# bjack205/altro

Measured on AMD Instinct MI355X. Metric: iLQR backward+forward sweeps/sec (N knotpoints x batch), higher is better.
Workload: dtype f64

## Files before the change

altro_amd/__init__.py:

```python
import ctypes as C
import os

import numpy as np

_HERE = os.path.dirname(os.path.abspath(__file__))
LIB_PATH = os.path.join(_HERE, "lib", "libaltro_hip.so")

F64, F32 = 0, 1
PLAN_AUTO, PLAN_GENERIC, PLAN_MFMA16, PLAN_LANE, PLAN_MFMA32 = 0, 1, 2, 3, 4
STORE_QBLOCKS = 0x1
LANE_FUSED = 0x4
F32_PURE = 0x2
TILE_USER_BLOCKS = 0x2
GENERIC_MATRIX_CORES = 0x8
TVLQR_SUCCESS = -1

C_ABI_SYMBOLS = [
    "altro_hip_version", "altro_hip_last_error", "altro_hip_device_count", "altro_hip_device_info", "altro_hip_device_pci_bus_id",
    "altro_hip_batch_create", "altro_hip_batch_create_dims", "altro_hip_batch_destroy", "altro_hip_batch_plan",
    "altro_hip_batch_device_bytes", "altro_hip_set_dynamics", "altro_hip_set_cost",
    "altro_hip_set_initial_state", "altro_hip_set_host_batch", "altro_hip_backward", "altro_hip_forward_ltv", "altro_hip_sweep",
    "altro_hip_synchronize", "altro_hip_get_K", "altro_hip_get_d", "altro_hip_get_P",
    "altro_hip_get_p", "altro_hip_get_x", "altro_hip_get_u", "altro_hip_get_y",
    "altro_hip_get_delta_V", "altro_hip_get_status", "altro_hip_get_qblocks",
    "altro_hip_stats_reduce", "altro_hip_comm_unique_id", "altro_hip_comm_create", "altro_hip_comm_create_all",
    "altro_hip_comm_destroy", "altro_hip_comm_rank", "altro_hip_comm_world", "altro_hip_comm_device", "altro_hip_stats_allreduce", "altro_hip_stats_allreduce_multi",
    "altro_hip_profile_enable", "altro_hip_profile_reset",
    "altro_hip_profile_get", "altro_hip_profile_get_range", "altro_hip_profile_dropped", "altro_hip_algorithmic_bytes",
    "altro_hip_set_model", "altro_hip_set_model_source", "altro_hip_model_row_layout", "altro_hip_set_tracking_cost", "altro_hip_set_quadratic_cost",
    "altro_hip_set_input_guess", "altro_hip_set_state_guess",
    "altro_hip_open_loop_rollout", "altro_hip_accept", "altro_hip_expand", "altro_hip_merit", "altro_hip_merit_affine",
    "altro_hip_stationarity", "altro_hip_get_nominal", "altro_hip_get_expansion",
    "altro_hip_default_solve_options", "altro_hip_set_forms", "altro_hip_get_forms", "altro_hip_ilqr_solve", "altro_hip_last_solve_counts",
    "altro_hip_ilqr_solve_async", "altro_hip_ilqr_poll", "altro_hip_ilqr_wait",
    "altro_hip_linesearch_host",
    "altro_hip_add_linear_constraint", "altro_hip_add_user_constraint", "altro_hip_clear_constraints", "altro_hip_reset_duals",
    "altro_hip_get_duals", "altro_hip_set_duals", "altro_hip_get_penalty", "altro_hip_set_penalty", "altro_hip_shift_duals", "altro_hip_feasibility",
    "altro_hip_shift_trajectory", "altro_hip_update_linear_costs", "altro_hip_get_knot",
    "altro_hip_set_pointer_mode",
]
CONE_EQUALITY, CONE_IDENTITY, CONE_INEQUALITY, CONE_SOC = 0, 1, 2, 3

DUAL_TAIL_KEEP, DUAL_TAIL_ZERO = 0, 1
FORM_NO_SPECULATION, FORM_NO_RUNAHEAD, FORM_NO_MERIT2, FORM_MERIT_LDS, FORM_MERIT_DPP_ALWAYS = 0x1, 0x2, 0x4, 0x8, 0x10
FORM_EXPAND_LDS, FORM_ALROWS_LDS, FORM_ROLLOUT_ROUNDS, FORM_SEQUENCED, FORM_MERIT_ONE_LAUNCH = 0x20, 0x40, 0x80, 0x100, 0x200
FORM_LANE_QUAD_OFF, FORM_LANE_QUAD_ON, FORM_GENERIC_LATE_Q_OFF, FORM_GENERIC_LATE_Q_ON, FORM_FUSED_CLOCK = 0x400, 0x800, 0x1000, 0x2000, 0x4000
FORM_AFFINE_EXACT = 0x8000
FORM_NO_COMPACTION = 0x10000
FORM_GENERIC_MERIT_LDS = 0x20000


def forms_from_env():
    e = os.environ
    off = lambda name: e.get(name) is not None and e[name].strip() not in ("",) and _atoi(e[name]) == 0
    f = 0
    if "ALTRO_HIP_NO_SPECULATION" in e: f |= FORM_NO_SPECULATION
    if "ALTRO_HIP_NO_RUNAHEAD" in e and not off("ALTRO_HIP_NO_RUNAHEAD"): f |= FORM_NO_RUNAHEAD
    if off("ALTRO_HIP_MERIT2"): f |= FORM_NO_MERIT2
    if off("ALTRO_HIP_MERIT_DPP"): f |= FORM_MERIT_LDS
    elif e.get("ALTRO_HIP_MERIT_DPP") is not None and _atoi(e["ALTRO_HIP_MERIT_DPP"]) == 2: f |= FORM_MERIT_DPP_ALWAYS
    if off("ALTRO_HIP_EXPAND_DPP"): f |= FORM_EXPAND_LDS
    if off("ALTRO_HIP_ALROWS_DPP"): f |= FORM_ALROWS_LDS
    if off("ALTRO_HIP_AFFINE"): f |= FORM_ROLLOUT_ROUNDS
    if off("ALTRO_HIP_FUSED") or "ALTRO_HIP_NO_FUSED" in e: f |= FORM_SEQUENCED
    if off("ALTRO_HIP_MERIT_SPLIT"): f |= FORM_MERIT_ONE_LAUNCH
    if "ALTRO_HIP_LANE_QUAD" in e: f |= FORM_LANE_QUAD_OFF if _atoi(e["ALTRO_HIP_LANE_QUAD"]) == 0 else FORM_LANE_QUAD_ON
    if "ALTRO_HIP_GENERIC_LATE_Q" in e: f |= FORM_GENERIC_LATE_Q_OFF if _atoi(e["ALTRO_HIP_GENERIC_LATE_Q"]) == 0 else FORM_GENERIC_LATE_Q_ON
    if "ALTRO_HIP_FUSED_CLOCK" in e: f |= FORM_FUSED_CLOCK
    if "ALTRO_HIP_AFFINE_EXACT" in e: f |= FORM_AFFINE_EXACT
    if "ALTRO_HIP_NO_COMPACTION" in e: f |= FORM_NO_COMPACTION
    return f


def _atoi(text):
    try:
        return int(text.strip() or 0)
    except ValueError:
        return 0

MODEL_LINEAR, MODEL_DOUBLE_INTEGRATOR, MODEL_PENDULUM, MODEL_BICYCLE, MODEL_USER, MODEL_QUADROTOR, MODEL_QUADROTOR13 = 0, 1, 2, 3, 4, 5, 6
MERIT_FN = C.CFUNCTYPE(None, C.c_double, C.POINTER(C.c_double), C.POINTER(C.c_double), C.c_void_p)

# ... 576 lines not shown
```

altro_amd/csrc/capi_core.hip:

```cpp
#include "capi_internal.h"

namespace altro_hip {
namespace capi {

thread_local std::string g_last_error;

int fail(int code, const char* fmt, ...) {
  char buf[512];
  va_list ap;
  va_start(ap, fmt);
  vsnprintf(buf, sizeof(buf), fmt, ap);
  va_end(ap);
  g_last_error = buf;
  return code;
}

}
}

using namespace altro_hip;
using namespace altro_hip::capi;

namespace {

// ... 581 lines not shown
  if (h->prof_n == 0) return 0;
  int rc = check(h);
  if (rc) return rc;
  HIP_TRY(hipStreamSynchronize(h->stream));
  for (int i = 0; i < h->prof_n; ++i) {
    float ms = 0.f;
    if (hipEventElapsedTime(&ms, h->prof_ev[2 * i], h->prof_ev[2 * i + 1]) != hipSuccess) continue;
    const int slot = h->prof_slot[i];
    h->prof_min[slot] = h->prof_launches[slot] ? std::min(h->prof_min[slot], (double)ms) : (double)ms;
    h->prof_max[slot] = std::max(h->prof_max[slot], (double)ms);
    h->prof_ms[slot] += ms;
    h->prof_launches[slot] += 1;
  }
  h->prof_n = 0;
  return 0;
}
}
int altro_hip_profile_get(altro_hip_batch* h, int slot, int* launches, double* total_ms,
                          const char** kernel_name) {
  if (!h || slot < 0 || slot > 1) return fail(ALTRO_HIP_ERR_BAD_ARGUMENT, "bad handle or slot");
  int rc = profile_drain(h);
  if (rc) return rc;
  if (launches) *launches = h->prof_launches[slot];
  if (total_ms) *total_ms = h->prof_ms[slot];
  if (kernel_name) {
    static const char* names[3][2] = {{"generic_backward_kernel", "generic_forward_kernel"},
                                      {"mfma16_backward_kernel", "mfma16_forward_kernel"},
                                      {"lane_backward_kernel", "lane_forward_kernel"}};
    *kernel_name = names[h->plan == ALTRO_HIP_PLAN_MFMA16 ? 1 : (h->plan == ALTRO_HIP_PLAN_LANE ? 2 : 0)][slot];
    if (h->g_tile && !(slot == 0 && h->is_diag)) *kernel_name = slot == 0 ? "tile32_backward_kernel" : "tile32_forward_kernel";
    if (slot == 0 && h->plan == ALTRO_HIP_PLAN_LANE && h->bwd_quad) *kernel_name = h->n == 4 ? "quad_backward_kernel" : "quad2_backward_kernel";
    if (slot == 1 && h->plan == ALTRO_HIP_PLAN_LANE && h->fwd_quad) *kernel_name = "quad_forward_kernel";
    if (slot == 1 && mfma16_forward_is_x4(h)) *kernel_name = "mfma16_forward_f32x4_kernel";
    if (slot == 0 && h->plan == ALTRO_HIP_PLAN_MFMA16 && h->dtype == ALTRO_HIP_F32 && (h->flags & ALTRO_HIP_F32_PURE) &&
        !(h->flags & ALTRO_HIP_STORE_QBLOCKS))
      *kernel_name = (h->batch % 4 == 0) ? "mfma16_backward_f32x4_kernel"
                                                                                    : "mfma16_backward_f32_kernel";
  }
  return 0;
}
int altro_hip_profile_dropped(altro_hip_batch* h, int slot) {
  if (!h || slot < 0 || slot > 1) return fail(ALTRO_HIP_ERR_BAD_ARGUMENT, "bad handle or slot");
  return h->prof_dropped[slot];
}
int altro_hip_profile_get_range(altro_hip_batch* h, int slot, double* min_ms, double* max_ms) {
  if (!h || slot < 0 || slot > 1) return fail(ALTRO_HIP_ERR_BAD_ARGUMENT, "bad handle or slot");
  int rc = profile_drain(h);
  if (rc) return rc;
  if (min_ms) *min_ms = h->prof_min[slot];
  if (max_ms) *max_ms = h->prof_max[slot];
  return 0;
}

double altro_hip_algorithmic_bytes(const altro_hip_batch* h, int slot) {
  if (!h) return 0.0;
  const double n = h->n, m = h->m, w = (double)h->esz;
  const double bwd = 3 * n * n + 3 * n * m + m * m + 3 * n + 2 * m;
  const double fwd = 2 * n * n + 2 * n * m + 4 * n + 2 * m;
  return (slot == 0 ? bwd : fwd) * w * (double)h->N * (double)h->batch;
}

}
```

altro_amd/csrc/capi_internal.h:

```cpp
#pragma once
#include "altro_hip/altro_hip.h"

#include <hip/hip_runtime.h>
#include <hip/hip_ext.h>

#include <algorithm>
#include <cstdarg>
#include <cstdio>
#include <cstdlib>
#include <cstring>
#include <string>
#include <vector>

#include "kernels/pack.hip"
#include "kernels/tvlqr_generic.hip"
#include "kernels/tvlqr_lane.hip"
#include "kernels/ilqr_types.h"
#include "kernels/ilqr_generic.hip"
#include "kernels/mfma16_layout.h"
#include "linesearch_sm.h"
#include "al_tables.h"
#include "al_shift.h"
#include "loop_fields.h"
#include "loop_route.h"
// ... 19 lines not shown

using namespace altro_hip;

struct altro_hip_batch {
  int N = 0, n = 0, m = 0, batch = 0, dtype = 0, plan = 0, device = 0;
  unsigned flags = 0;
  unsigned forms = 0;
  hipStream_t stream = nullptr;
  bool own_stream = false;
  size_t esz = 8;
  void* x0 = nullptr;
  void* delta_V = nullptr;
  int* status = nullptr;
  bool dyn_set = false, cost_set = false, x0_set = false, backward_done = false, forward_done = false;
  int has_f = 0, is_diag = 0;
  int host_batch = 0;
  bool dev_ptrs = false;
  void* g_arr[G_NUM] = {};
  int64_t g_bstride[G_NUM] = {};
  void *i_sens = nullptr, *i_sens_alpha = nullptr, *i_aff_part = nullptr, *i_aff_on = nullptr;
  bool aff_failed = false;
  bool aff_enabled = false, aff_round = false, aff_store = false;
  bool aff_base = false;
  bool g_tile = false;
  bool g_mfma = false;
  bool ragged = false;
  std::vector<int> nxv, nuv;
  int64_t* g_off = nullptr;
  int* g_nx = nullptr;
  int* g_nu = nullptr;
  void *m_in = nullptr, *m_cin = nullptr, *m_term = nullptr, *m_out = nullptr, *m_outn = nullptr, *m_xuy = nullptr,
       *m_qblk = nullptr, *m_trash = nullptr;
  Mfma16Strides m_st{};
  void *l_in = nullptr, *l_term = nullptr, *l_out = nullptr, *l_outn = nullptr, *l_xuy = nullptr,
       *l_x0 = nullptr;
  void *l_nom = nullptr, *l_cost = nullptr;
  IlqrProb* i_prob = nullptr;
  double *i_alpha = nullptr, *i_phi = nullptr, *i_dphi = nullptr;
  int *i_active = nullptr, *i_counters = nullptr;
  int* cnt_host = nullptr;
  int* cnt_host_dev = nullptr;
  hipEvent_t cnt_ev[16] = {};
  void* i_cand_spec = nullptr;
  void* poll_host = nullptr; int* poll_count_host = nullptr;
  bool async_request = false, async_pending = false;
  bool rtc_row32_ok = false;
  bool rtc_has_constraints = false;
  void* rtc = nullptr;
  std::string rtc_source;
  int rtc_ck = 0;
  int x0_stride = 0;
  int spare_count = 0;
  int spare_failed = 0;
  int *i_spec_sel = nullptr, *i_spec_refresh = nullptr;
  int* i_fused_list = nullptr;
  int fused_resident = 0;
  int *i_guard = nullptr, *i_active_exact = nullptr;
  int* i_stat_done = nullptr;
  const int* stat_skip = nullptr;
  void *i_merit_jk = nullptr, *i_spec_jac = nullptr;
  int merit_split = -1;
  void *i_results = nullptr, *i_results_host = nullptr;
  void* g_ws = nullptr;
  bool fwd_quad = false;
  bool bwd_quad = false;
  int spec_trials = 1;
// ... 385 lines not shown
inline int field_get(altro_hip_batch* h, const LoopShape& s, int field, int k0, int nk, double* host) {
  const FieldRef r = field_run(s, field, k0, &nk);
  if (r.kind == LK_LANE) return lane_get(h, host, loop_buffer(h, r.buf), k0 * r.ks, nullptr, r.E, (int)r.off, 0, r.len, nk, nk);
  return aos_get(h, host, loop_buffer(h, r.buf), r.off, r.bs, r.ks, r.len, nk);
}

constexpr int kCounterSlots = 2048;
constexpr int kStatsBlocks = 1024, kStatsStride = 16;

int rtc_current(altro_hip_batch* h, const RouteShape& s);
int rtc_step(altro_hip_batch* h, const RouteStep& st, const void* args);
RouteShape route_shape(const altro_hip_batch* h);

int replan_empty_handle(altro_hip_batch* h, int plan);
int al_upload(altro_hip_batch* h);
int model_takes_dynamics(altro_hip_batch* h);
int ilqr_check(altro_hip_batch* h, bool need_guess);
int ilqr_run(altro_hip_batch* h, int which, bool use_alpha, bool use_active, int want_deriv, double alpha_const,
             int mode = EXPAND_GRADIENT | EXPAND_HESSIAN);
template <typename T>
IlqrArgs<T> ilqr_args(altro_hip_batch* h, bool use_alpha, bool use_active, int want_deriv, double alpha_const);
int spec_trials_cap(const altro_hip_batch* h);
bool merit_rounds_dpp(const altro_hip_batch* h);
bool affine_eligible(const altro_hip_batch* h);
bool affine_buffers(altro_hip_batch* h);
bool ensure_spares(altro_hip_batch* h, int count, size_t bytes_each);
void merit_split_prepare(altro_hip_batch* h);
int ilqr_gather_results(altro_hip_batch* h, altro_hip_solve_result* results);
int launch_backward(altro_hip_batch* h, double reg);
bool tile32_supported(int n, int m);
int tile32_launch_backward(altro_hip_batch* h, double reg);
int tile32_launch_forward(altro_hip_batch* h);
int launch_forward(altro_hip_batch* h);
bool mfma16_forward_is_x4(const altro_hip_batch* h);

}
int al_shift_duals_launch(hipStream_t stream, void* z, int esz, const int* order, const int* start, int nchains, int batch, int tail);
int al_set_penalty_launch(hipStream_t stream, IlqrProb* prob, const double* rho, int stride, int batch);
int al_get_penalty_launch(hipStream_t stream, const IlqrProb* prob, double* rho, int batch);
namespace capi {

}
}
```

altro_amd/csrc/capi_tvlqr.hip:

```cpp
#include "capi_internal.h"
#include "models.h"

#include "kernels/tvlqr_mfma16.hip"
#include "kernels/tvlqr_mfma16_f32.hip"
#include "kernels/tvlqr_mfma16_f32x4.hip"
#include "kernels/tvlqr_mfma16_fwd_f32x4.hip"

using namespace altro_hip;
using namespace altro_hip::capi;

#define PROF_LAUNCH(kernel, grid, block, lds, stream, ...) \
  hipExtLaunchKernelGGL(kernel, grid, block, lds, stream, h->launch_ev0, h->launch_ev1, 0, __VA_ARGS__)

namespace {

template <typename T>
int lane_launch(altro_hip_batch* h, bool backward, double reg) {
  LaneArgs<T> a{(const T*)h->l_in, (const T*)h->l_term, (T*)h->l_out, (T*)h->l_outn, (const T*)h->l_x0,
                (T*)h->l_xuy, (T*)h->delta_V, h->status, h->N, h->batch, (T)reg, backward ? h->bwd_active : nullptr,
                backward ? h->bwd_reg : nullptr};
  const dim3 grid(8 * (((h->batch + 63) / 64 + 7) / 8)), block(64);
  const bool fused = (h->flags & ALTRO_HIP_LANE_FUSED) != 0;
  const bool quad_on = form(h, ALTRO_HIP_FORM_LANE_QUAD_ON) ? true : form(h, ALTRO_HIP_FORM_LANE_QUAD_OFF) ? false : h->batch <= 12288;
  const bool q42 = h->n == 4 && h->m == 2, q21 = h->n == 2 && h->m == 1;
  if (backward) h->bwd_quad = quad_on && (q42 || q21);
  if (!backward) h->fwd_quad = quad_on && q42;
  if (!backward && quad_on && q42) {
    const dim3 qgrid(8 * (((h->batch + 15) / 16 + 7) / 8));
    if (fused) PROF_LAUNCH((quad_forward_kernel_fused<2, T>), qgrid, block, 0, h->stream, a);
    else PROF_LAUNCH((quad_forward_kernel<2, T>), qgrid, block, 0, h->stream, a);
    hipError_t e = hipGetLastError();
    if (e != hipSuccess) return fail(ALTRO_HIP_ERR_HIP, "quad kernel launch: %s", hipGetErrorString(e));
    return 0;
  }
  if (backward && h->bwd_quad) {
    const dim3 qgrid(8 * (((h->batch + 15) / 16 + 7) / 8));
    if (q42 && fused) PROF_LAUNCH((quad_backward_kernel_fused<2, T>), qgrid, block, 0, h->stream, a);
    else if (q42) PROF_LAUNCH((quad_backward_kernel<2, T>), qgrid, block, 0, h->stream, a);
    else if (fused) PROF_LAUNCH((quad2_backward_kernel_fused<T>), qgrid, block, 0, h->stream, a);
// ... 73 lines not shown
    }
    h->launch_ev0 = nullptr; h->launch_ev1 = nullptr;
  }
};


template <typename S>
Mfma16Args<S> mfma16_args(altro_hip_batch* h, double reg) {
  Mfma16Args<S> a;
  a.in = (const S*)h->m_in;
  a.cin = (const S*)h->m_cin;
  a.cin_bs = h->m_st.cin_bs; a.cin_ks = h->m_st.cin_ks;
  a.in_bs = h->m_st.in_bs; a.in_ks = h->m_st.in_ks; a.out_bs = h->m_st.out_bs; a.out_ks = h->m_st.out_ks;
  a.xuy_bs = h->m_st.xuy_bs; a.xuy_ks = h->m_st.xuy_ks;
  a.term = (const S*)h->m_term; a.out = (S*)h->m_out; a.outn = (S*)h->m_outn; a.qblk = (S*)h->m_qblk;
  a.trash = (S*)h->m_trash; a.x0 = (const S*)h->x0; a.xuy = (S*)h->m_xuy; a.delta_V = (S*)h->delta_V;
  a.status = h->status; a.N = h->N; a.batch = h->batch; a.reg = reg; a.has_f = h->has_f && !h->ilqr_linear;
  a.active = h->bwd_active; a.reg_pp = h->bwd_reg;
  return a;
}
template <typename S>
void mfma16_launch_backward(altro_hip_batch* h, double reg, bool sq) {
  auto a = mfma16_args<S>(h, reg);
  const dim3 grid(mf_grid(h->batch)), block(64);
  if (sq && a.has_f) PROF_LAUNCH((mfma16_backward_kernel<true, true, S>), grid, block, 0, h->stream, a);
  else if (sq) PROF_LAUNCH((mfma16_backward_kernel<true, false, S>), grid, block, 0, h->stream, a);
  else if (a.has_f) PROF_LAUNCH((mfma16_backward_kernel<false, true, S>), grid, block, 0, h->stream, a);
  else PROF_LAUNCH((mfma16_backward_kernel<false, false, S>), grid, block, 0, h->stream, a);
}

template <typename S>
void mfma16_launch_forward(altro_hip_batch* h, const Mfma16Args<S>& a) {
  PROF_LAUNCH((mfma16_forward_kernel<S, 3>), dim3(mf_grid(h->batch)), dim3(64), 0, h->stream, a);
}

}

namespace altro_hip {
namespace capi {

int launch_backward(altro_hip_batch* h, double reg) {
  ProfScope ps(h, 0);
  h->aff_base = false;
  if (h->plan == ALTRO_HIP_PLAN_MFMA16) {
    const bool sq = (h->flags & ALTRO_HIP_STORE_QBLOCKS) != 0;
    if (h->dtype == ALTRO_HIP_F64) mfma16_launch_backward<double>(h, reg, sq);
    else if (sq || !(h->flags & ALTRO_HIP_F32_PURE)) mfma16_launch_backward<float>(h, reg, sq);
    else {
      auto a = mfma16_args<float>(h, reg);
      if (h->batch % 4 == 0) {
        const dim3 grid(mf_grid(h->batch / 4));
        if (a.has_f) PROF_LAUNCH((mfma16_backward_f32x4_kernel<true, 2, 2>), grid, dim3(64), 0, h->stream, a);
        else PROF_LAUNCH((mfma16_backward_f32x4_kernel<false, 2, 2>), grid, dim3(64), 0, h->stream, a);
      } else if (a.has_f) PROF_LAUNCH((mfma16_backward_f32_kernel<true, 3>), dim3(mf_grid(h->batch)), dim3(64), 0, h->stream, a);
      else PROF_LAUNCH((mfma16_backward_f32_kernel<false, 3>), dim3(mf_grid(h->batch)), dim3(64), 0, h->stream, a);
    }
  } else if (h->plan == ALTRO_HIP_PLAN_LANE) {
    return h->dtype == ALTRO_HIP_F64 ? lane_launch<double>(h, true, reg) : lane_launch<float>(h, true, reg);
  } else if (h->g_tile && !h->is_diag) {
    int rc = tile32_launch_backward(h, reg);
    if (rc) return rc;
  } else {
    const bool f64 = h->dtype == ALTRO_HIP_F64;
    const size_t lds4 = f64 ? generic_backward_lds_bytes<double>(h->n, h->m) : generic_backward_lds_bytes<float>(h->n, h->m);
    const size_t lds3 = f64 ? generic_backward_lds_bytes<double>(h->n, h->m, true) : generic_backward_lds_bytes<float>(h->n, h->m, true);
    const auto per_cu = [](size_t lds) { return (int)std::min<size_t>(16, (160 * 1024) / std::max<size_t>(lds, 1)); };
// ... 6 lines not shown
    const bool big = lds > kGenericLdsLimit;
    if (big && !h->g_ws) {
      int rc = dmalloc(h, &h->g_ws, (size_t)h->batch * ((lds + 15) / 16 * 16));
      if (rc) return rc;
    }
    if (f64) {
      auto a = generic_args<double>(h, reg);
      a.ws = (double*)h->g_ws; a.ws_stride = (int64_t)((lds + 15) / 16 * 16 / sizeof(double));
      const dim3 grid(h->batch), blk(64);
      if (h->g_mfma) {
        if (big) PROF_LAUNCH((generic_backward_kernel<double, true, true>), grid, blk, 0, h->stream, a);
        else if (late_q) PROF_LAUNCH((generic_backward_kernel<double, false, true, true>), grid, blk, lds, h->stream, a);
        else PROF_LAUNCH((generic_backward_kernel<double, false, true>), grid, blk, lds, h->stream, a);
      } else if (big) PROF_LAUNCH((generic_backward_kernel<double, true>), grid, blk, 0, h->stream, a);
      else if (late_q) PROF_LAUNCH((generic_backward_kernel<double, false, false, true>), grid, blk, lds, h->stream, a);
      else PROF_LAUNCH((generic_backward_kernel<double, false>), grid, blk, lds, h->stream, a);
    } else {
      auto a = generic_args<float>(h, reg);
      a.ws = (float*)h->g_ws; a.ws_stride = (int64_t)((lds + 15) / 16 * 16 / sizeof(float));
      if (big) PROF_LAUNCH((generic_backward_kernel<float, true>), dim3(h->batch), dim3(64), 0, h->stream, a);
      else if (late_q) PROF_LAUNCH((generic_backward_kernel<float, false, false, true>), dim3(h->batch), dim3(64), lds, h->stream, a);
      else PROF_LAUNCH((generic_backward_kernel<float, false>), dim3(h->batch), dim3(64), lds, h->stream, a);
    }
  }
  hipError_t e = hipGetLastError();
  if (e != hipSuccess) return fail(ALTRO_HIP_ERR_HIP, "backward launch: %s", hipGetErrorString(e));
  return 0;
}

bool mfma16_forward_is_x4(const altro_hip_batch* h) {
  return h->plan == ALTRO_HIP_PLAN_MFMA16 && h->dtype == ALTRO_HIP_F32 && (h->flags & ALTRO_HIP_F32_PURE) && h->batch % 4 == 0;
}

int launch_forward(altro_hip_batch* h) {
  ProfScope ps(h, 1);
  h->expansion_current = false;
  if (h->plan == ALTRO_HIP_PLAN_MFMA16) {
    if (h->dtype == ALTRO_HIP_F64) {
      auto a = mfma16_args<double>(h, 0.0);
      mfma16_launch_forward<double>(h, a);
    } else {
      auto a = mfma16_args<float>(h, 0.0);
      if (mfma16_forward_is_x4(h)) {
        const dim3 grid(mf_grid(h->batch / 4));
        PROF_LAUNCH((mfma16_forward_f32x4_kernel<2, 2>), grid, dim3(64), 0, h->stream, a);
      } else {
        mfma16_launch_forward<float>(h, a);
      }
    }
  } else if (h->plan == ALTRO_HIP_PLAN_LANE) {
    return h->dtype == ALTRO_HIP_F64 ? lane_launch<double>(h, false, 0.0) : lane_launch<float>(h, false, 0.0);
  } else if (h->g_tile) {
    int rc = tile32_launch_forward(h);
    if (rc) return rc;
  } else if (h->dtype == ALTRO_HIP_F64) {
    auto a = generic_args<double>(h, 0.0);
    const size_t staged = generic_forward_lds_bytes(h->n, h->m, a.want_y, sizeof(double));
    if (staged <= kGenericForwardStageLimit) PROF_LAUNCH((generic_forward_kernel<double, true>), dim3(h->batch), dim3(64), staged, h->stream, a);
    else PROF_LAUNCH((generic_forward_kernel<double, false>), dim3(h->batch), dim3(64), (size_t)(2 * h->n + h->m) * sizeof(double) + 64, h->stream, a);
  } else {
    auto a = generic_args<float>(h, 0.0);
    const size_t staged = generic_forward_lds_bytes(h->n, h->m, a.want_y, sizeof(float));
    if (staged <= kGenericForwardStageLimit) PROF_LAUNCH((generic_forward_kernel<float, true>), dim3(h->batch), dim3(64), staged, h->stream, a);
    else PROF_LAUNCH((generic_forward_kernel<float, false>), dim3(h->batch), dim3(64), (size_t)(2 * h->n + h->m) * sizeof(float) + 64, h->stream, a);
  }
  hipError_t e = hipGetLastError();
  if (e != hipSuccess) return fail(ALTRO_HIP_ERR_HIP, "forward launch: %s", hipGetErrorString(e));
  return 0;
}

}
}

// ... 110 lines not shown
```

altro_amd/csrc/kernels/tvlqr_mfma16.hip:

```cpp
#pragma once
#include <hip/hip_runtime.h>
#include <stdint.h>

#include "mfma16_layout.h"

namespace altro_hip {

typedef double f64x4 __attribute__((ext_vector_type(4)));

__device__ __forceinline__ f64x4 mfma_f64_16x16x4(double a, double b, f64x4 c) {
  return __builtin_amdgcn_mfma_f64_16x16x4f64(a, b, c, 0, 0, 0);
}

template <int CTRL>
__device__ __forceinline__ double dpp_mov_f64(double v) {
  union { double d; int i[2]; } in, out;
  in.d = v;
  out.i[0] = __builtin_amdgcn_update_dpp(in.i[0], in.i[0], CTRL, 0xf, 0xf, false);
  out.i[1] = __builtin_amdgcn_update_dpp(in.i[1], in.i[1], CTRL, 0xf, 0xf, false);
  return out.d;
}
__device__ __forceinline__ double row16_allreduce(double v) {
  v += dpp_mov_f64<0xB1>(v);
  v += dpp_mov_f64<0x4E>(v);
// ... 275 lines not shown
}
typedef float mf_f32x4 __attribute__((ext_vector_type(4)));
struct Mfma16FwdRegsF32 {
  mf_f32x4 dyn, out;
};
__device__ __forceinline__ void mfma16_fwd_load(Mfma16FwdRegsF32& r, const float* __restrict__ rec, const float* __restrict__ orec,
                                                int lane) {
  static_assert(MF_DYN % 4 == 0 && MF_OUT % 4 == 0 && MF_OFF_F % 4 == 0, "16-byte chunks never straddle a block");
  const int cd = lane < MF_DYN / 4 ? lane : MF_DYN / 4 - 1, co = lane < MF_OUT / 4 ? lane : MF_OUT / 4 - 1;
  r.dyn = *reinterpret_cast<const mf_f32x4*>(rec + 4 * cd);
  r.out = *reinterpret_cast<const mf_f32x4*>(orec + 4 * co);
}
__device__ __forceinline__ void mfma16_fwd_stage(const Mfma16FwdRegsF32& r, double* __restrict__ L, int lane) {
  const int cd = lane < MF_DYN / 4 ? lane : MF_DYN / 4 - 1, co = lane < MF_OUT / 4 ? lane : MF_OUT / 4 - 1;
  const int e = 4 * cd;
  const int base = e < MF_OFF_F ? (e >> 4) * MF_FWD_ZLD + (e & 15) : MF_FWD_F0 + (e - MF_OFF_F);
#pragma unroll
  for (int q = 0; q < 4; ++q) L[base + q] = (double)r.dyn[q];
#pragma unroll
  for (int q = 0; q < 4; ++q) L[MF_FWD_OUT0 + 4 * co + q] = (double)r.out[q];
}
template <typename S>
struct Mfma16FwdRing { using type = Mfma16FwdRegs; };
template <>
struct Mfma16FwdRing<float> { using type = Mfma16FwdRegsF32; };
__device__ __forceinline__ double readlane_f64(double v, int src_lane) {
  union { double d; int i[2]; } in, out;
  in.d = v;
  out.i[0] = __builtin_amdgcn_readlane(in.i[0], src_lane);
  out.i[1] = __builtin_amdgcn_readlane(in.i[1], src_lane);
  return out.d;
}

template <typename S, int DEPTH>
__global__ __launch_bounds__(64) void mfma16_forward_kernel(Mfma16Args<S> a) {
  __shared__ __attribute__((aligned(16))) double lds[MF_FWD_LDS + 4];
  __shared__ double xu_lds[16];
  const int lane = threadIdx.x;
  const int b = mf_problem(blockIdx.x, a.batch);
  if (b >= a.batch) return;
  const int N = a.N;
  const S* __restrict__ in = a.in + (size_t)b * a.in_bs;
  const S* __restrict__ out = a.out + (size_t)b * a.out_bs;
  S* __restrict__ xuy = a.xuy + (size_t)b * a.xuy_bs;
  S* __restrict__ trash = a.trash + (size_t)b * MF_OUT;
  const int grp = lane >> 4;
  const int sub = lane & 15;
  const int row = (grp == 1) ? (sub < 4 ? sub : 3) : (sub < 12 ? sub : 11);
  const int row_base = (grp == 0) ? MF_FWD_ZLD * row : MF_FWD_OUT0 + 13 * (grp == 1 ? row : 0);
  int ra[13];
#pragma unroll
  for (int jj = 0; jj < 12; ++jj) ra[jj] = (grp >= 2) ? MF_FWD_OUT0 + MF_OFF_P + mf_sym(row, jj) : row_base + jj;
  ra[12] = (grp >= 2) ? MF_FWD_OUT0 + MF_OFF_p + row : row_base + 12;
  const int out_off = (grp == 0) ? row : ((grp == 1) ? 24 + row : 12 + row);
  const bool is_x = (grp == 0), is_u = (grp == 1);

  double xcur = (double)a.x0[(size_t)b * 12 + row];
  typename Mfma16FwdRing<S>::type ring[DEPTH];
#pragma unroll
  for (int dd = 0; dd < DEPTH; ++dd) {
    const int kk = (dd < N) ? dd : N - 1;
    mfma16_fwd_load(ring[dd], in + (size_t)kk * a.in_ks, out + (size_t)kk * a.out_ks, lane);
  }
  __builtin_amdgcn_s_waitcnt(0x0F70);
  mfma16_fwd_stage(ring[0], lds, lane);
  __syncthreads();

  const int Npad = ((N + DEPTH - 1) / DEPTH) * DEPTH;
  for (int k0 = 0; k0 < Npad; k0 += DEPTH) {
#pragma unroll
    for (int dd = 0; dd < DEPTH; ++dd) {
      const int k = k0 + dd;
      const bool live = k < N;
      {
        const int kn = (k + DEPTH < N) ? k + DEPTH : N - 1;
        mfma16_fwd_load(ring[dd], in + (size_t)kn * a.in_ks, out + (size_t)kn * a.out_ks, lane);
      }
      double rd[16];
#pragma unroll
      for (int j = 0; j < 13; ++j) rd[j] = lds[ra[j]];
#pragma unroll
      for (int j = 13; j < 16; ++j) rd[j] = lds[row_base + j];
      const double fi = lds[MF_FWD_F0 + row];
      double xs[12];
      if constexpr (sizeof(S) == 4) {
        if (lane < 12) xu_lds[lane] = xcur;
        __builtin_amdgcn_s_waitcnt(0xC07F);
#pragma unroll
        for (int j = 0; j < 12; ++j) xs[j] = xu_lds[j];
      } else {
#pragma unroll
        for (int j = 0; j < 12; ++j) xs[j] = readlane_f64(xcur, j);
      }
      double acc = 0.0;
#pragma unroll
      for (int j = 0; j < 12; ++j) acc = __builtin_fma(rd[j], xs[j], acc);
      const double aff = acc + rd[12];
      const double uval = -aff;
      double us[4];
      if constexpr (sizeof(S) == 4) {
        if (lane >= 16 && lane < 20) xu_lds[lane - 4] = uval;
        __builtin_amdgcn_s_waitcnt(0xC07F);
#pragma unroll
        for (int c = 0; c < 4; ++c) us[c] = xu_lds[12 + c];
      } else {
#pragma unroll
        for (int c = 0; c < 4; ++c) us[c] = readlane_f64(uval, 16 + c);
      }
      double xn = acc + fi;
#pragma unroll
      for (int c = 0; c < 4; ++c) xn = __builtin_fma(rd[12 + c], us[c], xn);
      const double sval = is_x ? xcur : (is_u ? uval : aff);
      __syncthreads();
      mfma16_fwd_stage(ring[(dd + 1) % DEPTH], lds, lane);
      S* __restrict__ o = live ? xuy + (size_t)k * a.xuy_ks : trash;
      o[out_off] = (S)sval;
      __syncthreads();
      xcur = live ? xn : xcur;
    }
  }
  {
    const S* __restrict__ on = a.outn + (size_t)b * MF_TERM;
    double xs[12];
#pragma unroll
    for (int j = 0; j < 12; ++j) xs[j] = readlane_f64(xcur, j);
    double acc = (double)on[row * 13 + 12];
#pragma unroll
    for (int j = 0; j < 12; ++j) acc = __builtin_fma((double)on[row * 13 + j], xs[j], acc);
    const double sval = is_x ? xcur : (is_u ? 0.0 : acc);
    xuy[(size_t)N * a.xuy_ks + out_off] = (S)sval;
  }
}

__global__ void mfma16_selftest_kernel(const double* A, const double* B, const double* C, double* D) {
  const int lane = threadIdx.x, j = lane & 15, g = lane >> 4;
  f64x4 c;
#pragma unroll
  for (int r = 0; r < 4; ++r) c[r] = C[(g + 4 * r) * 16 + j];
  f64x4 d = mfma_f64_16x16x4(A[j * 4 + g], B[g * 16 + j], c);
#pragma unroll
  for (int r = 0; r < 4; ++r) D[(g + 4 * r) * 16 + j] = d[r];
}

}
```

include/altro_hip/altro_hip.h:

```cpp
#ifndef ALTRO_HIP_H_
#define ALTRO_HIP_H_

#include <stddef.h>
#include <stdint.h>

#ifdef __cplusplus
extern "C" {
#endif

#define ALTRO_HIP_VERSION 300
#define ALTRO_HIP_TVLQR_SUCCESS (-1)

typedef struct altro_hip_batch altro_hip_batch;

typedef enum altro_hip_dtype {
  ALTRO_HIP_F64 = 0,
  ALTRO_HIP_F32 = 1
} altro_hip_dtype;

typedef enum altro_hip_error {
  ALTRO_HIP_OK = 0,
  ALTRO_HIP_ERR_NO_DEVICE = -1,
  ALTRO_HIP_ERR_BAD_ARGUMENT = -2,
  ALTRO_HIP_ERR_UNSUPPORTED = -3,
// ... 110 lines not shown
  double tol_stationarity;
  double tol_primal_feasibility;
  double tol_meritfun_gradient;
  int use_backtracking_linesearch;
  double penalty_initial;
  double penalty_scaling;
  double penalty_max;
  double reg_initial;
  int reg_retry_max;
  double reg_scale, reg_min, reg_max;
  int stop_when_running_at_most;
  unsigned forms;
  int fused_sweeps;
  double decision_margin;
} altro_hip_solve_options;
#define ALTRO_HIP_FORM_NO_SPECULATION 0x0001u
#define ALTRO_HIP_FORM_NO_RUNAHEAD 0x0002u
#define ALTRO_HIP_FORM_NO_MERIT2 0x0004u
#define ALTRO_HIP_FORM_MERIT_LDS 0x0008u
#define ALTRO_HIP_FORM_MERIT_DPP_ALWAYS 0x0010u
#define ALTRO_HIP_FORM_EXPAND_LDS 0x0020u
#define ALTRO_HIP_FORM_ALROWS_LDS 0x0040u
#define ALTRO_HIP_FORM_ROLLOUT_ROUNDS 0x0080u
#define ALTRO_HIP_FORM_SEQUENCED 0x0100u
#define ALTRO_HIP_FORM_MERIT_ONE_LAUNCH 0x0200u
#define ALTRO_HIP_FORM_LANE_QUAD_OFF 0x0400u
#define ALTRO_HIP_FORM_LANE_QUAD_ON 0x0800u
#define ALTRO_HIP_FORM_GENERIC_LATE_Q_OFF 0x1000u
#define ALTRO_HIP_FORM_GENERIC_LATE_Q_ON 0x2000u
#define ALTRO_HIP_FORM_AFFINE_EXACT 0x8000u
#define ALTRO_HIP_FORM_FUSED_CLOCK 0x4000u
#define ALTRO_HIP_FORM_NO_COMPACTION 0x10000u
#define ALTRO_HIP_FORM_GENERIC_MERIT_LDS 0x20000u
int altro_hip_set_forms(altro_hip_batch* h, unsigned forms);
unsigned altro_hip_get_forms(const altro_hip_batch* h);
typedef struct altro_hip_solve_result {
  int status;
  int iterations;
  double stationarity;
  double final_alpha;
  double final_phi;
  double primal_feasibility;
  double penalty;
  int dual_updates;
  int reg_retries;
} altro_hip_solve_result;
void altro_hip_default_solve_options(altro_hip_solve_options* opts);
int altro_hip_ilqr_solve(altro_hip_batch* h, const altro_hip_solve_options* opts,
                         altro_hip_solve_result* results);
int altro_hip_last_solve_counts(const altro_hip_batch* h, int* sweeps, int* merit_launches);

typedef struct altro_hip_poll_record {
  altro_hip_solve_result result;
  double u0[4];
  int done;
  int reserved;
} altro_hip_poll_record;
int altro_hip_ilqr_solve_async(altro_hip_batch* h, const altro_hip_solve_options* opts);
int altro_hip_ilqr_poll(altro_hip_batch* h, int* n_done, const altro_hip_poll_record** records);
int altro_hip_ilqr_wait(altro_hip_batch* h, altro_hip_solve_result* results);

typedef void (*altro_hip_merit_fn)(double alpha, double* phi, double* dphi, void* ctx);
double altro_hip_linesearch_host(altro_hip_merit_fn f, void* ctx, double alpha0, double phi0, double dphi0,
                                 int try_cubic_first, int use_backtracking, double c1, double c2,
                                 int* status, int* iters, double* phi, double* dphi);

// ... 41 lines not shown
```

Before: 2.710 million.

## Add grouped fp64 MFMA16 forward kernel with cooperative coalesced record loads

Adds a forward-rollout kernel where 16 waves, each handling one batch problem, cooperatively load the contiguous dynamics and output records for all 16 problems as 16-byte chunks. The records go through a two-slot LDS ring with one block barrier per step, then each wave copies its own record into a private LDS image. This replaces per-wave strided loads with wide coalesced loads across adjacent batch entries. In exchange it adds block-wide barriers, larger dynamic LDS use and lower occupancy per block. It is selected by default for f64 MFMA16 when batch is a multiple of 16 and strides are packed; a new form flag restores the single-wave path, and the shared step code is factored into helpers.

Result: faster. 2.779 million (median of 6 runs) (+2.5%).

```diff
diff --git a/altro_amd/__init__.py b/altro_amd/__init__.py
--- a/altro_amd/__init__.py
+++ b/altro_amd/__init__.py
@@ -48,6 +48,7 @@
 FORM_AFFINE_EXACT = 0x8000
 FORM_NO_COMPACTION = 0x10000
 FORM_GENERIC_MERIT_LDS = 0x20000
+FORM_FORWARD_WAVE = 0x40000
 
 
 def forms_from_env():
diff --git a/altro_amd/csrc/capi_core.hip b/altro_amd/csrc/capi_core.hip
--- a/altro_amd/csrc/capi_core.hip
+++ b/altro_amd/csrc/capi_core.hip
@@ -637,6 +637,7 @@
     if (slot == 0 && h->plan == ALTRO_HIP_PLAN_LANE && h->bwd_quad) *kernel_name = h->n == 4 ? "quad_backward_kernel" : "quad2_backward_kernel";
     if (slot == 1 && h->plan == ALTRO_HIP_PLAN_LANE && h->fwd_quad) *kernel_name = "quad_forward_kernel";
     if (slot == 1 && mfma16_forward_is_x4(h)) *kernel_name = "mfma16_forward_f32x4_kernel";
+    if (slot == 1 && mfma16_forward_is_group(h)) *kernel_name = "mfma16_forward_group_kernel";
     if (slot == 0 && h->plan == ALTRO_HIP_PLAN_MFMA16 && h->dtype == ALTRO_HIP_F32 && (h->flags & ALTRO_HIP_F32_PURE) &&
         !(h->flags & ALTRO_HIP_STORE_QBLOCKS))
       *kernel_name = (h->batch % 4 == 0) ? "mfma16_backward_f32x4_kernel"
diff --git a/altro_amd/csrc/capi_internal.h b/altro_amd/csrc/capi_internal.h
--- a/altro_amd/csrc/capi_internal.h
+++ b/altro_amd/csrc/capi_internal.h
@@ -75,6 +75,7 @@
   void *m_in = nullptr, *m_cin = nullptr, *m_term = nullptr, *m_out = nullptr, *m_outn = nullptr, *m_xuy = nullptr,
        *m_qblk = nullptr, *m_trash = nullptr;
   Mfma16Strides m_st{};
+  bool fwd_group_ready = false;
   void *l_in = nullptr, *l_term = nullptr, *l_out = nullptr, *l_outn = nullptr, *l_xuy = nullptr,
        *l_x0 = nullptr;
   void *l_nom = nullptr, *l_cost = nullptr;
@@ -526,6 +527,7 @@
 int tile32_launch_backward(altro_hip_batch* h, double reg);
 int tile32_launch_forward(altro_hip_batch* h);
 int launch_forward(altro_hip_batch* h);
+bool mfma16_forward_is_group(const altro_hip_batch* h);
 bool mfma16_forward_is_x4(const altro_hip_batch* h);
 
 }
diff --git a/altro_amd/csrc/capi_tvlqr.hip b/altro_amd/csrc/capi_tvlqr.hip
--- a/altro_amd/csrc/capi_tvlqr.hip
+++ b/altro_amd/csrc/capi_tvlqr.hip
@@ -5,6 +5,7 @@
 #include "kernels/tvlqr_mfma16_f32.hip"
 #include "kernels/tvlqr_mfma16_f32x4.hip"
 #include "kernels/tvlqr_mfma16_fwd_f32x4.hip"
+#include "kernels/tvlqr_mfma16_fwd_group.hip"
 
 using namespace altro_hip;
 using namespace altro_hip::capi;
@@ -144,6 +145,19 @@
 template <typename S>
 void mfma16_launch_forward(altro_hip_batch* h, const Mfma16Args<S>& a) {
   PROF_LAUNCH((mfma16_forward_kernel<S, 3>), dim3(mf_grid(h->batch)), dim3(64), 0, h->stream, a);
+}
+
+constexpr int kFwdGroup = 16, kFwdGroupDepth = 2;
+int mfma16_launch_forward_group(altro_hip_batch* h, const Mfma16Args<double>& a) {
+  const auto kernel = mfma16_forward_group_kernel<double, kFwdGroup, kFwdGroupDepth>;
+  const size_t lds = Mfma16FwdGroup<kFwdGroup>::lds_bytes(kFwdGroupDepth);
+  if (!h->fwd_group_ready) {
+    hipError_t e = hipFuncSetAttribute((const void*)kernel, hipFuncAttributeMaxDynamicSharedMemorySize, (int)lds);
+    if (e != hipSuccess) return fail(ALTRO_HIP_ERR_HIP, "forward group kernel: %s", hipGetErrorString(e));
+    h->fwd_group_ready = true;
+  }
+  PROF_LAUNCH(kernel, dim3(mf_grid(h->batch / kFwdGroup)), dim3(64 * kFwdGroup), lds, h->stream, a);
+  return 0;
 }
 
 }
@@ -216,13 +230,25 @@
   return h->plan == ALTRO_HIP_PLAN_MFMA16 && h->dtype == ALTRO_HIP_F32 && (h->flags & ALTRO_HIP_F32_PURE) && h->batch % 4 == 0;
 }
 
+bool mfma16_forward_is_group(const altro_hip_batch* h) {
+  const int64_t B = h->batch;
+  return h->plan == ALTRO_HIP_PLAN_MFMA16 && h->dtype == ALTRO_HIP_F64 && !form(h, ALTRO_HIP_FORM_FORWARD_WAVE) &&
+         h->batch % kFwdGroup == 0 && h->m_st.in_bs == MF_DYN && h->m_st.in_ks == B * MF_DYN && h->m_st.out_bs == MF_OUT &&
+         h->m_st.out_ks == B * MF_OUT;
+}
+
 int launch_forward(altro_hip_batch* h) {
   ProfScope ps(h, 1);
   h->expansion_current = false;
   if (h->plan == ALTRO_HIP_PLAN_MFMA16) {
     if (h->dtype == ALTRO_HIP_F64) {
       auto a = mfma16_args<double>(h, 0.0);
-      mfma16_launch_forward<double>(h, a);
+      if (mfma16_forward_is_group(h)) {
+        int rc = mfma16_launch_forward_group(h, a);
+        if (rc) return rc;
+      } else {
+        mfma16_launch_forward<double>(h, a);
+      }
     } else {
       auto a = mfma16_args<float>(h, 0.0);
       if (mfma16_forward_is_x4(h)) {
diff --git a/altro_amd/csrc/kernels/tvlqr_mfma16.hip b/altro_amd/csrc/kernels/tvlqr_mfma16.hip
--- a/altro_amd/csrc/kernels/tvlqr_mfma16.hip
+++ b/altro_amd/csrc/kernels/tvlqr_mfma16.hip
@@ -331,6 +331,78 @@
   return out.d;
 }
 
+struct Mfma16FwdRole {
+  int row, row_base, out_off;
+  int ra[13];
+  bool is_x, is_u;
+};
+__device__ __forceinline__ Mfma16FwdRole mfma16_fwd_role(int lane) {
+  Mfma16FwdRole ro;
+  const int grp = lane >> 4;
+  const int sub = lane & 15;
+  ro.row = (grp == 1) ? (sub < 4 ? sub : 3) : (sub < 12 ? sub : 11);
+  ro.row_base = (grp == 0) ? MF_FWD_ZLD * ro.row : MF_FWD_OUT0 + 13 * (grp == 1 ? ro.row : 0);
+#pragma unroll
+  for (int jj = 0; jj < 12; ++jj) ro.ra[jj] = (grp >= 2) ? MF_FWD_OUT0 + MF_OFF_P + mf_sym(ro.row, jj) : ro.row_base + jj;
+  ro.ra[12] = (grp >= 2) ? MF_FWD_OUT0 + MF_OFF_p + ro.row : ro.row_base + 12;
+  ro.out_off = (grp == 0) ? ro.row : ((grp == 1) ? 24 + ro.row : 12 + ro.row);
+  ro.is_x = (grp == 0);
+  ro.is_u = (grp == 1);
+  return ro;
+}
+template <typename S>
+__device__ __forceinline__ double mfma16_fwd_step(const double* __restrict__ lds, double* __restrict__ xu_lds, const Mfma16FwdRole& ro,
+                                                  int lane, double xcur, S* __restrict__ o) {
+  double rd[16];
+#pragma unroll
+  for (int j = 0; j < 13; ++j) rd[j] = lds[ro.ra[j]];
+#pragma unroll
+  for (int j = 13; j < 16; ++j) rd[j] = lds[ro.row_base + j];
+  const double fi = lds[MF_FWD_F0 + ro.row];
+  double xs[12];
+  if constexpr (sizeof(S) == 4) {
+    if (lane < 12) xu_lds[lane] = xcur;
+    __builtin_amdgcn_s_waitcnt(0xC07F);
+#pragma unroll
+    for (int j = 0; j < 12; ++j) xs[j] = xu_lds[j];
+  } else {
+#pragma unroll
+    for (int j = 0; j < 12; ++j) xs[j] = readlane_f64(xcur, j);
+  }
+  double acc = 0.0;
+#pragma unroll
+  for (int j = 0; j < 12; ++j) acc = __builtin_fma(rd[j], xs[j], acc);
+  const double aff = acc + rd[12];
+  const double uval = -aff;
+  double us[4];
+  if constexpr (sizeof(S) == 4) {
+    if (lane >= 16 && lane < 20) xu_lds[lane - 4] = uval;
+    __builtin_amdgcn_s_waitcnt(0xC07F);
+#pragma unroll
+    for (int c = 0; c < 4; ++c) us[c] = xu_lds[12 + c];
+  } else {
+#pragma unroll
+    for (int c = 0; c < 4; ++c) us[c] = readlane_f64(uval, 16 + c);
+  }
+  double xn = acc + fi;
+#pragma unroll
+  for (int c = 0; c < 4; ++c) xn = __builtin_fma(rd[12 + c], us[c], xn);
+  const double sval = ro.is_x ? xcur : (ro.is_u ? uval : aff);
+  o[ro.out_off] = (S)sval;
+  return xn;
+}
+template <typename S>
+__device__ __forceinline__ void mfma16_fwd_terminal(const S* __restrict__ on, const Mfma16FwdRole& ro, double xcur, S* __restrict__ o) {
+  double xs[12];
+#pragma unroll
+  for (int j = 0; j < 12; ++j) xs[j] = readlane_f64(xcur, j);
+  double acc = (double)on[ro.row * 13 + 12];
+#pragma unroll
+  for (int j = 0; j < 12; ++j) acc = __builtin_fma((double)on[ro.row * 13 + j], xs[j], acc);
+  const double sval = ro.is_x ? xcur : (ro.is_u ? 0.0 : acc);
+  o[ro.out_off] = (S)sval;
+}
+
 template <typename S, int DEPTH>
 __global__ __launch_bounds__(64) void mfma16_forward_kernel(Mfma16Args<S> a) {
   __shared__ __attribute__((aligned(16))) double lds[MF_FWD_LDS + 4];
@@ -343,18 +415,9 @@
   const S* __restrict__ out = a.out + (size_t)b * a.out_bs;
   S* __restrict__ xuy = a.xuy + (size_t)b * a.xuy_bs;
   S* __restrict__ trash = a.trash + (size_t)b * MF_OUT;
-  const int grp = lane >> 4;
-  const int sub = lane & 15;
-  const int row = (grp == 1) ? (sub < 4 ? sub : 3) : (sub < 12 ? sub : 11);
-  const int row_base = (grp == 0) ? MF_FWD_ZLD * row : MF_FWD_OUT0 + 13 * (grp == 1 ? row : 0);
-  int ra[13];
-#pragma unroll
-  for (int jj = 0; jj < 12; ++jj) ra[jj] = (grp >= 2) ? MF_FWD_OUT0 + MF_OFF_P + mf_sym(row, jj) : row_base + jj;
-  ra[12] = (grp >= 2) ? MF_FWD_OUT0 + MF_OFF_p + row : row_base + 12;
-  const int out_off = (grp == 0) ? row : ((grp == 1) ? 24 + row : 12 + row);
-  const bool is_x = (grp == 0), is_u = (grp == 1);
-
-  double xcur = (double)a.x0[(size_t)b * 12 + row];
+  const Mfma16FwdRole ro = mfma16_fwd_role(lane);
+
+  double xcur = (double)a.x0[(size_t)b * 12 + ro.row];
   typename Mfma16FwdRing<S>::type ring[DEPTH];
 #pragma unroll
   for (int dd = 0; dd < DEPTH; ++dd) {
@@ -375,60 +438,15 @@
         const int kn = (k + DEPTH < N) ? k + DEPTH : N - 1;
         mfma16_fwd_load(ring[dd], in + (size_t)kn * a.in_ks, out + (size_t)kn * a.out_ks, lane);
       }
-      double rd[16];
-#pragma unroll
-      for (int j = 0; j < 13; ++j) rd[j] = lds[ra[j]];
-#pragma unroll
-      for (int j = 13; j < 16; ++j) rd[j] = lds[row_base + j];
-      const double fi = lds[MF_FWD_F0 + row];
-      double xs[12];
-      if constexpr (sizeof(S) == 4) {
-        if (lane < 12) xu_lds[lane] = xcur;
-        __builtin_amdgcn_s_waitcnt(0xC07F);
-#pragma unroll
-        for (int j = 0; j < 12; ++j) xs[j] = xu_lds[j];
-      } else {
-#pragma unroll
-        for (int j = 0; j < 12; ++j) xs[j] = readlane_f64(xcur, j);
-      }
-      double acc = 0.0;
-#pragma unroll
-      for (int j = 0; j < 12; ++j) acc = __builtin_fma(rd[j], xs[j], acc);
-      const double aff = acc + rd[12];
-      const double uval = -aff;
-      double us[4];
-      if constexpr (sizeof(S) == 4) {
-        if (lane >= 16 && lane < 20) xu_lds[lane - 4] = uval;
-        __builtin_amdgcn_s_waitcnt(0xC07F);
-#pragma unroll
-        for (int c = 0; c < 4; ++c) us[c] = xu_lds[12 + c];
-      } else {
-#pragma unroll
-        for (int c = 0; c < 4; ++c) us[c] = readlane_f64(uval, 16 + c);
-      }
-      double xn = acc + fi;
-#pragma unroll
-      for (int c = 0; c < 4; ++c) xn = __builtin_fma(rd[12 + c], us[c], xn);
-      const double sval = is_x ? xcur : (is_u ? uval : aff);
+      S* __restrict__ o = live ? xuy + (size_t)k * a.xuy_ks : trash;
+      const double xn = mfma16_fwd_step<S>(lds, xu_lds, ro, lane, xcur, o);
       __syncthreads();
       mfma16_fwd_stage(ring[(dd + 1) % DEPTH], lds, lane);
-      S* __restrict__ o = live ? xuy + (size_t)k * a.xuy_ks : trash;
-      o[out_off] = (S)sval;
       __syncthreads();
       xcur = live ? xn : xcur;
     }
   }
-  {
-    const S* __restrict__ on = a.outn + (size_t)b * MF_TERM;
-    double xs[12];
-#pragma unroll
-    for (int j = 0; j < 12; ++j) xs[j] = readlane_f64(xcur, j);
-    double acc = (double)on[row * 13 + 12];
-#pragma unroll
-    for (int j = 0; j < 12; ++j) acc = __builtin_fma((double)on[row * 13 + j], xs[j], acc);
-    const double sval = is_x ? xcur : (is_u ? 0.0 : acc);
-    xuy[(size_t)N * a.xuy_ks + out_off] = (S)sval;
-  }
+  mfma16_fwd_terminal<S>(a.outn + (size_t)b * MF_TERM, ro, xcur, xuy + (size_t)N * a.xuy_ks);
 }
 
 __global__ void mfma16_selftest_kernel(const double* A, const double* B, const double* C, double* D) {
diff --git a/altro_amd/csrc/kernels/tvlqr_mfma16_fwd_group.hip b/altro_amd/csrc/kernels/tvlqr_mfma16_fwd_group.hip
--- /dev/null
+++ b/altro_amd/csrc/kernels/tvlqr_mfma16_fwd_group.hip
@@ -0,0 +1,94 @@
+#pragma once
+#include "tvlqr_mfma16.hip"
+
+namespace altro_hip {
+
+typedef double mf_f64x2 __attribute__((ext_vector_type(2)));
+
+template <int G>
+struct Mfma16FwdGroup {
+  static constexpr int T = 64 * G;
+  static constexpr int CD = MF_DYN / 2, CO = MF_OUT / 2;
+  static constexpr int CIN = G * (CD + CO);
+  static constexpr int ROUNDS = (CIN + T - 1) / T;
+  static constexpr int SLOT = CIN;
+  static constexpr int IMG = MF_FWD_LDS + 4;
+  static constexpr size_t lds_bytes(int depth) { return ((size_t)depth * SLOT * 2 + (size_t)G * IMG) * sizeof(double); }
+};
+static_assert(MF_DYN % 2 == 0 && MF_OUT % 2 == 0, "records are whole 16-byte chunks");
+
+template <typename S, int G, int DEPTH>
+__global__ __launch_bounds__(64 * G) void mfma16_forward_group_kernel(Mfma16Args<S> a) {
+  static_assert(sizeof(S) == 8, "fp64 records (handles that store fp32 keep their own kernels)");
+  static_assert(DEPTH >= 2, "one barrier per step needs two ring slots");
+  using GR = Mfma16FwdGroup<G>;
+  static_assert(GR::lds_bytes(DEPTH) <= 160 * 1024, "LDS of one CU");
+  extern __shared__ __attribute__((aligned(16))) double mf_fwd_group_lds[];
+  mf_f64x2* const ring = (mf_f64x2*)mf_fwd_group_lds;
+  const int t = threadIdx.x, lane = t & 63;
+  const int wv = __builtin_amdgcn_readfirstlane(t >> 6);
+  double* const img = mf_fwd_group_lds + (size_t)DEPTH * GR::SLOT * 2 + (size_t)wv * GR::IMG;
+  const int ngrp = a.batch / G;
+  const int grp = mf_problem(blockIdx.x, ngrp);
+  if (grp >= ngrp) return;
+  const int b0 = grp * G, b = b0 + wv;
+  const int N = a.N;
+  S* __restrict__ xuy = a.xuy + (size_t)b * a.xuy_bs;
+  S* __restrict__ trash = a.trash + (size_t)b * MF_OUT;
+  const Mfma16FwdRole ro = mfma16_fwd_role(lane);
+
+  const mf_f64x2* src[GR::ROUNDS];
+  int64_t sstride[GR::ROUNDS];
+  int dst[GR::ROUNDS];
+#pragma unroll
+  for (int r = 0; r < GR::ROUNDS; ++r) {
+    int c = r * GR::T + t;
+    c = c < GR::CIN ? c : GR::CIN - 1;
+    dst[r] = c;
+    const bool dyn = c < G * GR::CD;
+    src[r] = dyn ? (const mf_f64x2*)(a.in + (size_t)b0 * MF_DYN) + c : (const mf_f64x2*)(a.out + (size_t)b0 * MF_OUT) + (c - G * GR::CD);
+    sstride[r] = (dyn ? a.in_ks : a.out_ks) / 2;
+  }
+  mf_f64x2 regs[DEPTH][GR::ROUNDS];
+  auto fetch = [&](mf_f64x2* rg, int k) {
+    const int64_t kk = k < N ? k : N - 1;
+#pragma unroll
+    for (int r = 0; r < GR::ROUNDS; ++r) rg[r] = src[r][kk * sstride[r]];
+  };
+
+  double xcur = (double)a.x0[(size_t)b * 12 + ro.row];
+#pragma unroll
+  for (int dd = 0; dd < DEPTH; ++dd) fetch(regs[dd], dd);
+  __builtin_amdgcn_s_waitcnt(0x0F70);
+
+  const int Npad = ((N + DEPTH - 1) / DEPTH) * DEPTH;
+  for (int k0 = 0; k0 < Npad; k0 += DEPTH) {
+#pragma unroll
+    for (int dd = 0; dd < DEPTH; ++dd) {
+      const int k = k0 + dd;
+      const bool live = k < N;
+      mf_f64x2* const slot = ring + dd * GR::SLOT;
+#pragma unroll
+      for (int r = 0; r < GR::ROUNDS; ++r) slot[dst[r]] = regs[dd][r];
+      fetch(regs[dd], k + DEPTH);
+      asm volatile("s_waitcnt lgkmcnt(0)" ::: "memory");
+      __builtin_amdgcn_s_barrier();
+      asm volatile("" ::: "memory");
+      {
+        const double* __restrict__ rec = (const double*)slot + wv * MF_DYN;
+        const double* __restrict__ orec = (const double*)slot + G * MF_DYN + wv * MF_OUT;
+        Mfma16FwdRegs rr;
+        mfma16_fwd_load(rr, rec, orec, lane);
+        mfma16_fwd_stage(rr, img, lane);
+      }
+      asm volatile("s_waitcnt lgkmcnt(0)" ::: "memory");
+      __builtin_amdgcn_wave_barrier();
+      S* __restrict__ o = live ? xuy + (size_t)k * a.xuy_ks : trash;
+      const double xn = mfma16_fwd_step<S>(img, nullptr, ro, lane, xcur, o);
+      xcur = live ? xn : xcur;
+    }
+  }
+  mfma16_fwd_terminal<S>(a.outn + (size_t)b * MF_TERM, ro, xcur, xuy + (size_t)N * a.xuy_ks);
+}
+
+}
diff --git a/include/altro_hip/altro_hip.h b/include/altro_hip/altro_hip.h
--- a/include/altro_hip/altro_hip.h
+++ b/include/altro_hip/altro_hip.h
@@ -166,6 +166,7 @@
 #define ALTRO_HIP_FORM_FUSED_CLOCK 0x4000u
 #define ALTRO_HIP_FORM_NO_COMPACTION 0x10000u
 #define ALTRO_HIP_FORM_GENERIC_MERIT_LDS 0x20000u
+#define ALTRO_HIP_FORM_FORWARD_WAVE 0x40000u
 int altro_hip_set_forms(altro_hip_batch* h, unsigned forms);
 unsigned altro_hip_get_forms(const altro_hip_batch* h);
 typedef struct altro_hip_solve_result {
```
